# theovincent/iS-DQN

Hardware: AMD Instinct MI355X
Metric: gradient-steps/sec (batch=256, K=9, 84x84x4) (higher is better)
Workload: dtype bf16x3 (split-bf16 MFMA operands hi+lo, fp32 accumulate)

## Files before the change

__graft_entry__.py:

```python
import importlib.util
import os
import sys

ROOT = os.path.dirname(os.path.abspath(__file__))
PKG = os.path.join(ROOT, "is-dqn_amd")
for _p in (ROOT, PKG):
    if _p not in sys.path:
        sys.path.insert(0, _p)


def _build_module():
    spec = importlib.util.spec_from_file_location("isdqn_build", os.path.join(PKG, "build.py"))
    mod = importlib.util.module_from_spec(spec)
    spec.loader.exec_module(mod)
    return mod


def build() -> None:
    from concurrent.futures import ThreadPoolExecutor

    mod = _build_module()
    with ThreadPoolExecutor(4) as pool:
        jobs = [pool.submit(mod.build, verbose=True),
                pool.submit(mod.build, verbose=True, variant="bounds", defines=("ISDQN_BOUNDS",)),
                pool.submit(mod.build, verbose=True, variant="nopair", defines=("ISDQN_NO_U8_PAIR",)),
                pool.submit(mod.build, verbose=True, variant="dev", defines=("ISDQN_DEV",))]
        lib_path = jobs[0].result()
        for j in jobs[1:]:
            j.result()
    from slimdqn import _hip

    handle = _hip.lib()
    for name in _hip.PUBLIC_SYMBOLS:
        getattr(handle, name)
    import slimdqn.networks.isdqn
    import slimdqn.sample_collection.replay_buffer
    import slimdqn.sample_collection.samplers
    import slimdqn.sample_collection.sum_tree

    print(f"built {lib_path}: {handle.isdqn_version().decode()}")


def smoke() -> None:
    import numpy as np
    import torch

    from oracle.isdqn import iSDQN as Oracle
    from oracle.replay_buffer import ReplayBuffer as ORB, TransitionElement as OT
    from oracle.samplers import PrioritizedSamplingDistribution as OP
    from slimdqn.networks.isdqn import iSDQN
    from slimdqn.sample_collection.replay_buffer import ReplayBuffer, TransitionElement
    from slimdqn.sample_collection.samplers import PrioritizedSamplingDistribution

    assert torch.cuda.is_available(), "smoke() needs a GPU"
    K, A, B, feats = 3, 6, 8, [16, 16, 16, 32]
    agent = iSDQN(0, (84, 84, 4), A, K, feats, True, False, "cnn", 1e-3, 0.99, 3, 1, 4, adam_eps=1.5e-4, batch_size=B)
    oracle = Oracle(0, (84, 84, 4), A, K, feats, True, False, "cnn", 1e-3, 0.99, 3, 1, 4, adam_eps=1.5e-4,
                    params=agent.get_model()["params"]["params"])
    rb = ReplayBuffer(PrioritizedSamplingDistribution(1, 64), B, 64, update_horizon=3, gamma=0.99)
# ... 24 lines not shown
```

is-dqn_amd/csrc/gemm_core.h:

```cpp
#pragma once
#include <cstdio>
#include <cstdlib>
#include <type_traits>
#include "common.h"

namespace isdqn {

typedef __attribute__((ext_vector_type(8))) __bf16 bf16x8;
typedef __attribute__((ext_vector_type(4))) short s16x4;
typedef __attribute__((ext_vector_type(8))) short s16x8;
typedef __attribute__((ext_vector_type(4))) float f32x4;

constexpr int GEMM_BK = 32;
constexpr int GEMM_THREADS = 256;

__device__ __forceinline__ int xcd_remap(int bid, int n_blocks) {
    const int xcd = bid & 7, q = n_blocks >> 3, r = n_blocks & 7;
    const int base = xcd < r ? xcd * (q + 1) : r * (q + 1) + (xcd - r) * q;
    return base + (bid >> 3);
}

#define LDS_AS __attribute__((address_space(3)))

__device__ __forceinline__ void split8(const float (&v)[8], bf16x8& hi, bf16x8& lo) {
// ... 106 lines not shown
    if constexpr (!TR) {
        return *reinterpret_cast<const bf16x8*>(tile + (row0 + (lane & 15)) * PITCH + (lane >> 4) * 8);
    } else {
        const int g = lane >> 4, i = lane & 15, q = i >> 2, p = i & 3;
        const __bf16* a0 = tile + (16 * (g >> 1) + 2 * q + (g & 1)) * PITCH + row0 + 4 * p;
        const __bf16* a1 = a0 + 8 * PITCH;
        s16x4 lo = __builtin_amdgcn_ds_read_tr16_b64_v4i16((LDS_AS s16x4*)a0);
        s16x4 hi = __builtin_amdgcn_ds_read_tr16_b64_v4i16((LDS_AS s16x4*)a1);
        s16x8 r = __builtin_shufflevector(lo, hi, 0, 1, 2, 3, 4, 5, 6, 7);
        return __builtin_bit_cast(bf16x8, r);
    }
}

template <class P, class = void>
struct KGroupsOf { static constexpr int value = 1; };
template <class P>
struct KGroupsOf<P, std::void_t<decltype(P::KG)>> { static constexpr int value = P::KG; };
template <class P, class = void>
struct TrPadAOf { static constexpr int value = 16; };
template <class P>
struct TrPadAOf<P, std::void_t<decltype(P::TR_PAD_A)>> { static constexpr int value = P::TR_PAD_A; };
template <class P, class = void>
struct TrPadBOf { static constexpr int value = 16; };
template <class P>
struct TrPadBOf<P, std::void_t<decltype(P::TR_PAD_B)>> { static constexpr int value = P::TR_PAD_B; };
template <class P, class = void>
struct AS8Of { static constexpr bool value = false; };
template <class P>
struct AS8Of<P, std::void_t<decltype(P::A_S8)>> { static constexpr bool value = P::A_S8; };
template <class P, class = void>
struct BS8Of { static constexpr bool value = false; };
template <class P>
struct BS8Of<P, std::void_t<decltype(P::B_S8)>> { static constexpr bool value = P::B_S8; };

template <class P>
struct GemmTraits {
    static constexpr int BM = P::BM, BN = P::BN, WM = P::WM, WN = P::WN;
    static constexpr int MT = BM / WM / 16, NT = BN / WN / 16;
    static constexpr int PASSES = P::PASSES;
    static constexpr int A_PLANES = PASSES >= 2 ? 2 : 1;
    static constexpr int B_PLANES = PASSES >= 3 ? 2 : 1;
    using GA = TileGeom<BM, P::A_TR, TrPadAOf<P>::value>;
    using GB = TileGeom<BN, P::B_TR, TrPadBOf<P>::value>;
    static constexpr int STAGE_ELEMS = A_PLANES * GA::ELEMS + B_PLANES * GB::ELEMS;
    static constexpr int KG = KGroupsOf<P>::value;
    static constexpr int PIPE_BYTES = KG * 2 * STAGE_ELEMS * 2;
    static constexpr int XCHG_BYTES = KG > 1 ? KG * 4 * NT * 4 * 64 * 4 : 0;
    static constexpr int EPI_BYTES = P::EPI_LDS_BYTES + XCHG_BYTES;
    static constexpr int LDS_BYTES = PIPE_BYTES > EPI_BYTES ? PIPE_BYTES : EPI_BYTES;
};

template <class P>
__global__ __launch_bounds__(GEMM_THREADS * KGroupsOf<P>::value) void gemm_kernel(const P p) {
    ISDQN_EMPTY_KERNEL_RETURN
    using T = GemmTraits<P>;
    constexpr int KG = T::KG;
    using GA = typename T::GA;
    using GB = typename T::GB;
    constexpr int MT = T::MT, NT = T::NT, PASSES = T::PASSES;
    extern __shared__ __attribute__((aligned(16))) char smem_raw[];
    __bf16* smem = reinterpret_cast<__bf16*>(smem_raw);

    typename P::Tile tile;
    if (!p.tile((int)blockIdx.x, tile)) return;

    const int kg = KG > 1 ? (int)threadIdx.x / GEMM_THREADS : 0;
    const int tid = (int)threadIdx.x - kg * GEMM_THREADS;
    const int lane = tid & 63;
    const int wave = tid >> 6;
    const int wm = wave / P::WN, wn = wave % P::WN;
    const int wave_m = wm * (MT * 16), wave_n = wn * (NT * 16);

    typename P::ACtx actx[GA::PER_THREAD];
    typename P::BCtx bctx[GB::PER_THREAD];
    int a_lds[GA::PER_THREAD], a_var[GA::PER_THREAD];
    int b_lds[GB::PER_THREAD], b_var[GB::PER_THREAD];
    bool a_on[GA::PER_THREAD], b_on[GB::PER_THREAD];
#pragma unroll
    for (int i = 0; i < GA::PER_THREAD; ++i) {
        int c = tid + i * GEMM_THREADS;
        a_on[i] = c < GA::CHUNKS;
        if (!a_on[i]) c = 0;
        if constexpr (!P::A_TR) {
            int r = stash_row(c), kc = c & 3;
            actx[i] = p.a_ctx(tile, tile.m0 + r);
            a_var[i] = kc * 8;
            a_lds[i] = r * GA::PITCH + kc * 8;
        } else {
            int kk = c / (T::BM / 8), rc = c % (T::BM / 8);
            actx[i] = p.a_ctx(tile, tile.m0 + rc * 8);
            a_var[i] = kk;
            a_lds[i] = tr_row(kk) * GA::PITCH + rc * 8;
        }
    }
#pragma unroll
    for (int i = 0; i < GB::PER_THREAD; ++i) {
// ... 59 lines not shown
#pragma unroll
    for (int mt = 0; mt < MT; ++mt)
#pragma unroll
        for (int nt = 0; nt < NT; ++nt) mfma_init(acc[mt][nt]);

    auto compute = [&](int stage) {
        const __bf16* base = smem + (kg * 2 + stage) * T::STAGE_ELEMS;
        const __bf16* a_hi = base;
        const __bf16* a_lo = base + GA::ELEMS;
        const __bf16* b_hi = base + T::A_PLANES * GA::ELEMS;
        const __bf16* b_lo = b_hi + GB::ELEMS;
        bf16x8 fa_hi[MT], fa_lo[MT];
#pragma unroll
        for (int mt = 0; mt < MT; ++mt) {
            fa_hi[mt] = read_frag<P::A_TR, GA::PITCH>(a_hi, wave_m + mt * 16, lane);
            if constexpr (PASSES >= 2) fa_lo[mt] = read_frag<P::A_TR, GA::PITCH>(a_lo, wave_m + mt * 16, lane);
        }
#pragma unroll
        for (int nt = 0; nt < NT; ++nt) {
            bf16x8 fb_hi = read_frag<P::B_TR, GB::PITCH>(b_hi, wave_n + nt * 16, lane);
            bf16x8 fb_lo;
            if constexpr (PASSES >= 3) fb_lo = read_frag<P::B_TR, GB::PITCH>(b_lo, wave_n + nt * 16, lane);
#pragma unroll
            for (int mt = 0; mt < MT; ++mt) {
                if constexpr (PASSES >= 3)
                    mfma_acc(acc[mt][nt], fa_hi[mt], fb_lo);
                if constexpr (PASSES >= 2)
                    mfma_acc(acc[mt][nt], fa_lo[mt], fb_hi);
                mfma_acc(acc[mt][nt], fa_hi[mt], fb_hi);
            }
        }
    };

    const int nsteps = ((tile.k1 - tile.k0 + GEMM_BK - 1) / GEMM_BK + KG - 1) / KG;
    if (nsteps > 0) {
        fetch(tile.k0 + kg * GEMM_BK);
        stash(0);
        __syncthreads();
        for (int s = 0; s < nsteps; ++s) {
            const bool more = s + 1 < nsteps;
            if (more) fetch(tile.k0 + ((s + 1) * KG + kg) * GEMM_BK);
            compute(s & 1);
            if (more) stash((s + 1) & 1);
            __syncthreads();
        }
    }
    if constexpr (KG > 1) {
        static_assert(KG == 2 && MT == 2, "one row tile per K group");
        float* red = reinterpret_cast<float*>(smem_raw + P::EPI_LDS_BYTES);
#pragma unroll
        for (int nt = 0; nt < NT; ++nt)
#pragma unroll
            for (int r = 0; r < 4; ++r) {
                const float give = kg == 0 ? acc[1][nt][r] : acc[0][nt][r];
                red[(((kg * 4 + wave) * NT + nt) * 4 + r) * 64 + lane] = give;
            }
        __syncthreads();
        f32x4 mine[1][NT];
#pragma unroll
        for (int nt = 0; nt < NT; ++nt)
#pragma unroll
            for (int r = 0; r < 4; ++r) {
                const float got = red[((((1 - kg) * 4 + wave) * NT + nt) * 4 + r) * 64 + lane];
                mine[0][nt][r] = (kg == 0 ? acc[0][nt][r] : acc[1][nt][r]) + got;
            }
        p.epilogue(tile, mine, tile.m0 + wave_m + kg * 16, tile.n0 + wave_n, lane, smem_raw);
    } else {
        p.epilogue(tile, acc, tile.m0 + wave_m, tile.n0 + wave_n, lane, smem_raw);
    }
}

template <class P>
static int launch_gemm(const P& p, int n_blocks, hipStream_t stream) {
    using T = GemmTraits<P>;
    static LdsConfigured configured;
    int rc = ensure_dynamic_lds(&gemm_kernel<P>, T::LDS_BYTES, configured);
    if (rc) return rc;
    ISDQN_REPORT_OCCUPANCY((&gemm_kernel<P>), GEMM_THREADS * T::KG, T::LDS_BYTES, n_blocks);
    if (n_blocks <= 0) return ISDQN_OK;
    hipLaunchKernelGGL(gemm_kernel<P>, dim3(n_blocks), dim3(GEMM_THREADS * T::KG), T::LDS_BYTES, stream, p);
    ISDQN_HIP_CHECK(hipGetLastError());
    return ISDQN_OK;
}

__device__ __forceinline__ void zero8(float (&v)[8]) {
#pragma unroll
    for (int i = 0; i < 8; ++i) v[i] = 0.f;
}
__device__ __forceinline__ float row16_sum(float x) {
    auto dpp = [](float v, auto ctrl) {
        return __builtin_bit_cast(float, __builtin_amdgcn_update_dpp(0, __builtin_bit_cast(int, v), decltype(ctrl)::value, 0xF, 0xF, true));
    };
    x += dpp(x, std::integral_constant<int, 0xB1>{});
    x += dpp(x, std::integral_constant<int, 0x4E>{});
    x += dpp(x, std::integral_constant<int, 0x124>{});
    x += dpp(x, std::integral_constant<int, 0x128>{});
    return x;
}

static __device__ const float isdqn_zero_block[16] = {0.f, 0.f, 0.f, 0.f, 0.f, 0.f, 0.f, 0.f,
                                                      0.f, 0.f, 0.f, 0.f, 0.f, 0.f, 0.f, 0.f};
__device__ __forceinline__ const float* zero_chunk() { return isdqn_zero_block; }

#if defined(ISDQN_BOUNDS)
struct BoundsTable {
    int n, bad, bad_site, pad;
    unsigned long long bad_addr;
    unsigned long long lo[64], hi[64];
};
static __device__ BoundsTable isdqn_bounds;
__device__ __forceinline__ void bounds_check(const void* p, int bytes, int site) {
    const unsigned long long a = (unsigned long long)p, b = a + (unsigned)bytes;
    const unsigned long long z = (unsigned long long)isdqn_zero_block;
// ... 71 lines not shown
```

is-dqn_amd/csrc/learn_step.h:

```cpp
#pragma once
struct SideStream {
    hipStream_t stream = nullptr;
    hipEvent_t ev[2 * MAX_LAYERS + 4];
    int n_ev = 0;
    std::atomic<unsigned> next{0};
    std::atomic<int> state{0};
};
static SideStream* side_stream() {
    static SideStream per_dev[ISDQN_MAX_DEVICES];
    if (ISDQN_DEV_ENV("ISDQN_SINGLE_STREAM")) return nullptr;
    SideStream& s = per_dev[current_device_slot()];
    int st = s.state.load(std::memory_order_acquire);
    if (st == 2) return &s;
    if (st == -1) return nullptr;
    int expected = 0;
    if (s.state.compare_exchange_strong(expected, 1)) {
        bool ok = hipStreamCreateWithFlags(&s.stream, hipStreamNonBlocking) == hipSuccess;
        s.n_ev = 2 * MAX_LAYERS + 4;
        for (int i = 0; ok && i < s.n_ev; ++i) ok = hipEventCreateWithFlags(&s.ev[i], hipEventDisableTiming) == hipSuccess;
        s.state.store(ok ? 2 : -1, std::memory_order_release);
        return ok ? &s : nullptr;
    }
    while ((st = s.state.load(std::memory_order_acquire)) == 1) {}
    return st == 2 ? &s : nullptr;
// ... 139 lines not shown
static int learn_loss(const LearnCtx& c) {
    const bool tnet = (c.double_q || c.munchausen) && c.target_params != nullptr;
    if (!c.hc_S) {
        int rc = loss_and_finalize(c.P, c, c.double_q, tnet ? c.ws + c.P.out_t_off + (c.munchausen ? (int64_t)c.B * c.P.nlog_p : 0) : nullptr,
                                   (tnet && c.munchausen) ? c.ws + c.P.out_t_off : nullptr);
        if (rc || !(c.learn() && c.P.dueling)) return rc;
        const Plan& P = c.P;
        const int w = P.head_nb > 0 ? P.head_nb : 1;
        const int64_t threads = (int64_t)(c.B + 1) * P.n_heads * w;
        hipLaunchKernelGGL(duel_backward_kernel, dim3((unsigned)((threads + DUEL_THREADS - 1) / DUEL_THREADS)), dim3(DUEL_THREADS), 0, c.st,
                           (const float*)(c.ws + P.dout_off), P.nlog_p, c.ws + P.dout_raw_off, P.raw_p, (const float*)(c.ws + P.dbh_off),
                           c.ws + P.dbh_raw_off, c.B, P.n_heads, P.n_actions, w);
        ISDQN_HIP_CHECK(hipGetLastError());
        return ISDQN_OK;
    }
    if (int rc = launch_head_chain(c)) return rc;
    return c.ss ? ISDQN_OK : head_chain_sums(c, c.st);
}

struct WgradJob {
    int layer = -1;
    hipStream_t stream = nullptr;
    hipEvent_t wait = nullptr;
    const float* dz = nullptr;
    int dz_ld = 0;
};

static int dense_wgrad_fused_adam(const LearnCtx& c, const Layer& l, const float* act_in, const WgradJob& j) {
    const MatSrc A{j.dz, j.dz_ld, c.B, l.out_p, 1};
    const MatSrc Bm{act_in, l.in_p, c.B, l.in_p, 1};
    AdamFuse af{c.params + l.w_off, c.adam_m + l.w_off, c.adam_v + l.w_off, c.ws + c.P.adam_tab_off,
                c.cfg->learning_rate, c.cfg->adam_b1, c.cfg->adam_b2, c.cfg->adam_eps,
                c.grad_out ? c.grad_out + l.w_off : nullptr, c.ws + c.P.wsplit_off + l.w_off, c.update() ? 1 : 0, c.wd(1)};
    if (l.is_head)
        return c.x3 ? launch_plain<64, 64, 2, 2, true, true, 3, true, false, true, 2>(A, nullptr, 0, Bm, nullptr, l.in_p, l.out_p, l.in_p, c.B, 1, 0,
                                                                                      j.stream, &af)
                    : launch_plain<64, 64, 2, 2, true, true, 1, true, false, true, 2>(A, nullptr, 0, Bm, nullptr, l.in_p, l.out_p, l.in_p, c.B, 1, 0,
                                                                                      j.stream, &af);
    return c.x3 ? launch_plain<64, 64, 2, 2, true, true, 3, true, false, true, DZ_S8 | 2>(A, nullptr, 0, Bm, nullptr, l.in_p, l.out_p, l.in_p, c.B, 1,
                                                                                          0, j.stream, &af)
                : launch_plain<64, 64, 2, 2, true, true, 1, true, false, true, DZ_S8 | 2>(A, nullptr, 0, Bm, nullptr, l.in_p, l.out_p, l.in_p, c.B, 1,
                                                                                          0, j.stream, &af);
}

static int weight_gradient(const LearnCtx& c, const WgradJob& j, AdamList* adam) {
    const Layer& l = c.P.L[j.layer];
    float* ws = c.ws;
    const float* act_in = j.layer > 0 ? ws + c.P.L[j.layer - 1].act_off : nullptr;
    int w_slabs, rc;
    if (l.is_head && c.hc_S && c.ss) {
        w_slabs = effective_splits(c.B, l.gw_slabs);
    } else if (l.kind == 0) {
        rc = conv_wgrad(l, c.x3, c.in, act_in, j.dz, ws + l.gw_off, c.B, j.stream, &w_slabs);
        if (rc) return rc;
    } else {
        w_slabs = effective_splits(c.B, l.gw_slabs);
        if (w_slabs == 1 && !l.in_unpadded_ld && !c.P.grad_clip) return dense_wgrad_fused_adam(c, l, act_in, j);
        rc = dense_wgrad(l, c.x3, c.in, act_in, j.dz, j.dz_ld, ws + l.gw_off, c.B, j.stream);
        if (rc) return rc;
    }
    adam[c.ss && j.stream == c.wst ? 1 : 0].add(l.w_off, l.w_size, ws + l.gw_off, w_slabs, l.w_size, c.wd(l.kind == 0 ? 0 : 1));
    return ISDQN_OK;
}

#if !defined(ISDQN_FORK_LATE_MAX_B)
#define ISDQN_FORK_LATE_MAX_B 768
#endif
struct BackwardSchedule {
    const LearnCtx& c;
    AdamList* const adam;
    const bool tail_swap, fork_late;
    bool prio_pending, head_pending;
    hipEvent_t head_event = nullptr;
    bool forked = false, layer0_chained = false;
    WgradJob deferred;
// ... 324 lines not shown
```

is-dqn_amd/csrc/net_launch.h:

```cpp
#pragma once
#if defined(ISDQN_DEV)
static long long* g_stamps = nullptr;
static int g_stamp_layer = -1;
static char g_stamp_name[32] = "";
extern "C" int isdqn_debug_set_stamps(void* buf, const char* layer_name) {
    g_stamps = (long long*)buf;
    g_stamp_layer = buf ? 0 : -1;
    snprintf(g_stamp_name, sizeof(g_stamp_name), "%s", layer_name ? layer_name : "");
    return ISDQN_OK;
}
static long long* stamps_for(const char* kernel_tag) {
    return (g_stamp_layer >= 0 && strcmp(kernel_tag, g_stamp_name) == 0) ? g_stamps : nullptr;
}
#else
static long long* stamps_for(const char*) { return nullptr; }
#endif

__global__ __launch_bounds__(256) void split_params_kernel(const float* __restrict__ p, float* __restrict__ mirror, int64_t n_groups) {
    const int64_t g = (int64_t)blockIdx.x * 256 + threadIdx.x;
    if (g >= n_groups) return;
    float v[8];
    load8_aligned(p + g * 8, v);
    s8_store_group(mirror + g * 8, v);
}
// ... 110 lines not shown
    if (passes == 3) return mt == 2 ? launch_conv_fwd_img<2, 3, false>(ip, st)
                          : kg2 ? launch_conv_fwd_img<4, 3, false, 2>(ip, st) : launch_conv_fwd_img<4, 3, false>(ip, st);
    return mt == 2 ? launch_conv_fwd_img<2, 1, false>(ip, st)
         : kg2 ? launch_conv_fwd_img<4, 1, false, 2>(ip, st) : launch_conv_fwd_img<4, 1, false>(ip, st);
}

static int conv_fwd(const Layer& l, bool x3, const float* params, const float* wmir, const NetInput& in, const float* act_in, int n_img,
                    int z_img, float* act, float* z, hipStream_t st) {
    bool done = false;
    int rc = conv_fwd_img(l, x3, params, wmir, in, act_in, n_img, z_img, act, z, st, &done);
    if (rc || done) return rc;
    const bool small = l.cout_p <= 32;
    if (l.is_u8) {
        if (x3) return small ? launch_conv_fwd<32, 2, true>(l, params, wmir, in, act_in, n_img, z_img, act, z, st)
                             : launch_conv_fwd<64, 2, true>(l, params, wmir, in, act_in, n_img, z_img, act, z, st);
        return small ? launch_conv_fwd<32, 1, true>(l, params, wmir, in, act_in, n_img, z_img, act, z, st)
                     : launch_conv_fwd<64, 1, true>(l, params, wmir, in, act_in, n_img, z_img, act, z, st);
    }
    if (x3) return small ? launch_conv_fwd<32, 3, false>(l, params, wmir, in, act_in, n_img, z_img, act, z, st)
                         : launch_conv_fwd<64, 3, false>(l, params, wmir, in, act_in, n_img, z_img, act, z, st);
    return small ? launch_conv_fwd<32, 1, false>(l, params, wmir, in, act_in, n_img, z_img, act, z, st)
                 : launch_conv_fwd<64, 1, false>(l, params, wmir, in, act_in, n_img, z_img, act, z, st);
}

static int effective_splits(int K, int splits, int* steps_per_split = nullptr) {
    int ksteps = ceil_div(K, GEMM_BK);
    if (splits < 1) splits = 1;
    if (splits > ksteps) splits = ksteps;
    int sps = ceil_div(ksteps, splits);
    if (steps_per_split) *steps_per_split = sps;
    return ceil_div(ksteps, sps);
}

template <int BM, int BN, int WM, int WN, bool ATR, bool BTR, int PASSES, bool AL, bool A2PART, bool ADAM = false, int S8M = 0>
static int launch_plain(const MatSrc& A, const float* A2, int a_split, const MatSrc& B, float* C, int ldc, int M,
                        int N, int K, int splits, int64_t slab_stride, hipStream_t st,
                        const AdamFuse* adam = nullptr) {
    PlainGemm<BM, BN, WM, WN, ATR, BTR, PASSES, AL, A2PART, ADAM, S8M> p;
    if (adam) p.adam = *adam;
    p.A = A; p.B = B; p.A2 = A2; p.a_split = a_split; p.C = C; p.ldc = ldc; p.M = M; p.N = N; p.K = K;
    p.tiles_m = ceil_div(M, BM); p.tiles_n = ceil_div(N, BN);
    p.splits = effective_splits(K, splits, &p.steps_per_split);
    p.slab_stride = slab_stride;
    return launch_gemm(p, p.tiles_m * p.tiles_n * p.splits, st);
}

template <bool ATR, bool BTR, bool AL = true, bool A2PART = false, int S8M = 0>
static int plain_big(bool x3, const MatSrc& A, const float* A2, int a_split, const MatSrc& B, float* C, int ldc,
                     int M, int N, int K, int splits, int64_t slab_stride, hipStream_t st) {
    if (x3)
        return launch_plain<128, 128, 2, 2, ATR, BTR, 3, AL, A2PART, false, S8M>(A, A2, a_split, B, C, ldc, M, N, K, splits,
                                                                                 slab_stride, st);
    return launch_plain<128, 128, 2, 2, ATR, BTR, 1, AL, A2PART, false, S8M>(A, A2, a_split, B, C, ldc, M, N, K, splits,
                                                                             slab_stride, st);
}

template <bool ATR, bool BTR, int S8M = 0>
static int plain_narrow(bool x3, const MatSrc& A, const MatSrc& B, float* C, int ldc, int M, int N, int K, int splits,
                        int64_t slab_stride, hipStream_t st) {
    if (x3) return launch_plain<128, 64, 2, 2, ATR, BTR, 3, true, false, false, S8M>(A, nullptr, 0, B, C, ldc, M, N, K, splits, slab_stride, st);
    return launch_plain<128, 64, 2, 2, ATR, BTR, 1, true, false, false, S8M>(A, nullptr, 0, B, C, ldc, M, N, K, splits, slab_stride, st);
}

static int dense_fwd(const Layer& l, bool x3, const float* params, const float* wmir, const NetInput& in, const float* act_in, int rows,
                     int z_rows, float* slab, float* act, float* z, hipStream_t st, bool skip_post = false) {
    MatSrc A, B;
    const float* A2 = nullptr;
    int a_split = 0;
    if (l.in_unpadded_ld) {
        A = MatSrc{in.obs, l.in_unpadded_ld, rows, l.in_f, 0};
        if (in.obs2) { A2 = in.obs2; a_split = in.obs_split; }
    } else {
        A = MatSrc{act_in, l.in_p, rows, l.in_p, 1};
    }
    B = MatSrc{wmir + l.w_off, l.in_p, l.out_f, l.in_p, 1};
    const int ns = effective_splits(l.in_unpadded_ld ? l.in_f : l.K, l.fwd_splits);
    const int64_t slab_stride = l.out_p;
// ... 520 lines not shown
```

is-dqn_amd/csrc/net_problems.h:

```cpp
#pragma once
#include "gemm_core.h"

namespace isdqn {

struct FrameSrc {
    const uint8_t* frames;
    int64_t stride;
    const int* ids;
    int stack;
    int paired_B;
    int H, W;
    int id_pitch = 0, id_off = 0;
    __device__ __forceinline__ int frame_id(int j, int c) const {
#if defined(ISDQN_DEV)
        if (ids == nullptr) return j * stack + c;
#endif
        if (paired_B > 0) {
            const int* q = j < paired_B ? ids + (int64_t)j * 2 * stack + c : ids + (int64_t)(j - paired_B) * 2 * stack + stack + c;
            ISDQN_BOUNDS_CHECK(q, 4, 4);
            return *q;
        }
        ISDQN_BOUNDS_CHECK(ids + (int64_t)j * (id_pitch ? id_pitch : stack) + id_off + c, 4, 4);
        return ids[(int64_t)j * (id_pitch ? id_pitch : stack) + id_off + c];
    }
// ... 20 lines not shown
        patch8_cvt(u, d, v);
    }
    __device__ __forceinline__ void patch8(int j, int c, int iy, int ix0, float (&v)[8]) const {
        patch8_id(frame_id(j, c), iy, ix0, v);
    }
};

struct AdamFuse {
    float *p, *m, *v;
    const float* consts;
    float lr, b1, b2, eps;
    float* grad_out;
    float* mirror;
    int update;
    float wd = 0.f;
};

template <int BM_, int BN_, int WM_, int WN_, bool ATR, bool BTR, int PASSES_, bool AL = true, bool A2PART = false,
          bool ADAM = false, int S8M = 0>
struct PlainGemm {
    static constexpr int BM = BM_, BN = BN_, WM = WM_, WN = WN_, PASSES = PASSES_;
    static constexpr bool A_TR = ATR, B_TR = BTR;
    static constexpr bool A_S8 = (S8M & 1) != 0, B_S8 = (S8M & 2) != 0;
    static constexpr int TR_PAD_B = ADAM ? 8 : 16;
    MatSrc A, B;
    const float* A2;
    int a_split;
    float* C;
    int ldc, M, N, K;
    int tiles_m, tiles_n, splits, steps_per_split;
    int64_t slab_stride;
    AdamFuse adam;
    static constexpr int EPI_LDS_BYTES = ADAM ? BM_ * (BN_ + 4) * 4 : 0;
    struct Tile { int m0, n0, k0, k1, split; };
    struct ACtx { int fixed; };
    struct BCtx { int fixed; };
    __device__ __forceinline__ bool tile(int bid, Tile& t) const {
        bid = xcd_remap(bid, tiles_m * tiles_n * splits);
        int tm = bid % tiles_m, rest = bid / tiles_m;
        int tn = rest % tiles_n;
        t.split = rest / tiles_n;
#if defined(ISDQN_ADAM_ROWMAJOR)
        if constexpr (ADAM) {
            tn = bid % tiles_n;
            tm = bid / tiles_n;
        }
#endif
        if (t.split >= splits) return false;
        t.m0 = tm * BM;
        t.n0 = tn * BN;
        t.k0 = t.split * steps_per_split * GEMM_BK;
        t.k1 = min(K, t.k0 + steps_per_split * GEMM_BK);
        return true;
    }
    __device__ __forceinline__ ACtx a_ctx(const Tile&, int fixed) const { return ACtx{fixed}; }
    __device__ __forceinline__ BCtx b_ctx(const Tile&, int fixed) const { return BCtx{fixed}; }
    __device__ __forceinline__ void load_a(const Tile&, const ACtx& c, int var, float (&v)[8]) const {
        if constexpr (!ATR) {
            if constexpr (A2PART) {
                const bool second = c.fixed >= a_split;
                MatSrc s = A;
                s.base = second ? A2 : A.base;
                s.outer = second ? A.outer - a_split : min(A.outer, a_split);
                s.load<AL || A_S8>(second ? c.fixed - a_split : c.fixed, var, v);
            } else {
                A.load<AL || A_S8>(c.fixed, var, v);
            }
        } else {
            A.load<AL || A_S8>(var, c.fixed, v);
        }
    }
    __device__ __forceinline__ void load_b(const Tile&, const BCtx& c, int var, float (&v)[8]) const {
        if constexpr (!BTR) B.load<AL || B_S8>(c.fixed, var, v);
        else B.load<AL || B_S8>(var, c.fixed, v);
    }
    template <int MT, int NT>
    __device__ __forceinline__ void epilogue(const Tile& t, f32x4 (&acc)[MT][NT], int m_wave, int n_wave, int lane, char* smem) const {
        if constexpr (ADAM) {
            constexpr int LD = BN + 4;
            float* tg = reinterpret_cast<float*>(smem);
            const int lm = m_wave - t.m0, ln = n_wave - t.n0;
            constexpr int N_IT = BM * (BN / 4) / GEMM_THREADS;
            static_assert(BM * (BN / 4) % GEMM_THREADS == 0, "whole float4 rounds");
            const int tid = threadIdx.x;
            f32x4 pm[N_IT], pv[N_IT], pp[N_IT];
            int64_t off[N_IT];
            bool on[N_IT];
#pragma unroll
            for (int it = 0; it < N_IT; ++it) {
                const int i = tid + it * GEMM_THREADS;
                const int rl = i / (BN / 4), c4 = (i % (BN / 4)) * 4;
                const int row = t.m0 + rl, col = t.n0 + c4;
                on[it] = row < M && col < N;
                off[it] = on[it] ? (int64_t)row * ldc + col : 0;
                ISDQN_BOUNDS_CHECK(adam.m + off[it], 16, 10);
                ISDQN_BOUNDS_CHECK(adam.v + off[it], 16, 10);
                ISDQN_BOUNDS_CHECK(adam.p + off[it], 16, 10);
#if !defined(ISDQN_NO_STREAMING)
                pm[it] = __builtin_nontemporal_load((const ISDQN_GLOBAL f32x4*)(adam.m + off[it]));
                pv[it] = __builtin_nontemporal_load((const ISDQN_GLOBAL f32x4*)(adam.v + off[it]));
                pp[it] = __builtin_nontemporal_load((const ISDQN_GLOBAL f32x4*)(adam.p + off[it]));
#else
                pm[it] = *(const ISDQN_GLOBAL f32x4*)(adam.m + off[it]);
                pv[it] = *(const ISDQN_GLOBAL f32x4*)(adam.v + off[it]);
                pp[it] = *(const ISDQN_GLOBAL f32x4*)(adam.p + off[it]);
#endif
            }
#pragma unroll
            for (int mt = 0; mt < MT; ++mt)
#pragma unroll
                for (int nt = 0; nt < NT; ++nt)
#pragma unroll
                    for (int r = 0; r < 4; ++r)
                        tg[(lm + mt * 16 + (lane >> 4) * 4 + r) * LD + ln + nt * 16 + (lane & 15)] = acc[mt][nt][r];
            __syncthreads();
            const float inv_c1 = 1.f / adam.consts[0], inv_c2 = 1.f / adam.consts[1];
#pragma unroll
            for (int it = 0; it < N_IT; ++it) {
                const int i = tid + it * GEMM_THREADS;
                const int rl = i / (BN / 4), c4 = (i % (BN / 4)) * 4;
                const float4 g = *reinterpret_cast<const float4*>(tg + rl * LD + c4);
                const float* gp = &g.x;
                f32x4 nm, nv, np;
#pragma unroll
                for (int r = 0; r < 4; ++r) {
                    float mm = pm[it][r], vv = pv[it][r];
                    np[r] = adam_element(mm, vv, pp[it][r], gp[r], adam.b1, adam.b2, adam.lr, adam.eps, inv_c1, inv_c2);
                    nm[r] = mm;
                    nv[r] = vv;
                }
                if (adam.wd != 0.f) {
#pragma unroll
                    for (int r = 0; r < 4; ++r) np[r] = adamw_decay(np[r], pp[it][r], adam.lr, adam.wd);
                }
                if (on[it] && adam.grad_out) *reinterpret_cast<float4*>(adam.grad_out + off[it]) = g;
                if (on[it] && adam.update) {
#if !defined(ISDQN_NO_STREAMING)
                    __builtin_nontemporal_store(nm, (ISDQN_GLOBAL f32x4*)(adam.m + off[it]));
                    __builtin_nontemporal_store(nv, (ISDQN_GLOBAL f32x4*)(adam.v + off[it]));
                    __builtin_nontemporal_store(np, (ISDQN_GLOBAL f32x4*)(adam.p + off[it]));
#else
                    *reinterpret_cast<f32x4*>(adam.m + off[it]) = nm;
                    *reinterpret_cast<f32x4*>(adam.v + off[it]) = nv;
                    *reinterpret_cast<f32x4*>(adam.p + off[it]) = np;
#endif
                    s8_store_quad(adam.mirror, (int)off[it], np[0], np[1], np[2], np[3]);
                }
            }
            return;
        }
        float* c = C + (int64_t)t.split * slab_stride;
#pragma unroll
        for (int mt = 0; mt < MT; ++mt)
#pragma unroll
            for (int nt = 0; nt < NT; ++nt) {
                int col = n_wave + nt * 16 + (lane & 15);
#pragma unroll
                for (int r = 0; r < 4; ++r) {
                    int row = m_wave + mt * 16 + (lane >> 4) * 4 + r;
                    if (row < M && col < N) c[(int64_t)row * ldc + col] = acc[mt][nt][r];
                }
            }
    }
};

template <int PASSES_, int BM_ = 128, int KG_ = 1>
struct DenseDgradLN {
    static constexpr int BM = BM_, BN = 64, WM = 4, WN = 1, PASSES = PASSES_;
    static constexpr int KG = KG_;
    static constexpr bool A_TR = false, B_TR = true;
    static constexpr bool A_S8 = true;
    static constexpr bool B_S8 = true;
    static constexpr int TR_PITCH = 68;
    static constexpr int SP_BYTES = 4 * KG_ * 3 * 64 * 4;
    static constexpr int EPI_LDS_BYTES = SP_BYTES + 4 * KG_ * 16 * TR_PITCH * 4;
    MatSrc A, B;
    const float* z;
    const float *gamma, *beta;
    float* dz_out;
    float* part;
    int ldc, M, N, K, c_in;
// ... 423 lines not shown
```

Before: 4366.

## Make Adam-fused weight-gradient GEMM persistent and interleave Adam state prefetch with K-loop

The Adam-fused GEMM becomes a persistent kernel. A capped grid, about one workgroup per CU, loops over tiles. The Adam m/v/p state loads are spread across the first K-loop iterations instead of being issued all at once in the epilogue. This aims to hide the optimizer-state memory latency behind MFMA work and to cut launch/tail overhead from many small tiles. In exchange, LDS grows when the epilogue and pipeline buffers are separate, and register pressure rises from holding the prefetched state.

```diff
diff --git a/__graft_entry__.py b/__graft_entry__.py
--- a/__graft_entry__.py
+++ b/__graft_entry__.py
@@ -20,11 +20,12 @@
     from concurrent.futures import ThreadPoolExecutor
 
     mod = _build_module()
-    with ThreadPoolExecutor(4) as pool:
+    with ThreadPoolExecutor(5) as pool:
         jobs = [pool.submit(mod.build, verbose=True),
                 pool.submit(mod.build, verbose=True, variant="bounds", defines=("ISDQN_BOUNDS",)),
                 pool.submit(mod.build, verbose=True, variant="nopair", defines=("ISDQN_NO_U8_PAIR",)),
-                pool.submit(mod.build, verbose=True, variant="dev", defines=("ISDQN_DEV",))]
+                pool.submit(mod.build, verbose=True, variant="dev", defines=("ISDQN_DEV",)),
+                pool.submit(mod.build, verbose=True, variant="adam1t", defines=("ISDQN_ADAM_ONE_TILE",))]
         lib_path = jobs[0].result()
         for j in jobs[1:]:
             j.result()
diff --git a/is-dqn_amd/csrc/gemm_core.h b/is-dqn_amd/csrc/gemm_core.h
--- a/is-dqn_amd/csrc/gemm_core.h
+++ b/is-dqn_amd/csrc/gemm_core.h
@@ -162,6 +162,11 @@
 struct BS8Of { static constexpr bool value = false; };
 template <class P>
 struct BS8Of<P, std::void_t<decltype(P::B_S8)>> { static constexpr bool value = P::B_S8; };
+
+template <class P, class = void>
+struct PersistentOf { static constexpr bool value = false; };
+template <class P>
+struct PersistentOf<P, std::void_t<decltype(P::PERSISTENT)>> { static constexpr bool value = P::PERSISTENT; };
 
 template <class P>
 struct GemmTraits {
@@ -177,8 +182,20 @@
     static constexpr int PIPE_BYTES = KG * 2 * STAGE_ELEMS * 2;
     static constexpr int XCHG_BYTES = KG > 1 ? KG * 4 * NT * 4 * 64 * 4 : 0;
     static constexpr int EPI_BYTES = P::EPI_LDS_BYTES + XCHG_BYTES;
-    static constexpr int LDS_BYTES = PIPE_BYTES > EPI_BYTES ? PIPE_BYTES : EPI_BYTES;
+    static constexpr bool PERSIST = PersistentOf<P>::value;
+    static constexpr int LDS_SHARED_BYTES = PIPE_BYTES > EPI_BYTES ? PIPE_BYTES : EPI_BYTES;
+    static constexpr int LDS_BYTES = PERSIST ? PIPE_BYTES + EPI_BYTES : LDS_SHARED_BYTES;
 };
+
+#if defined(ISDQN_DEV)
+#define ISDQN_GEMM_STAMP(cond, slot)                                                                             \
+    if ((cond) && p.stamps != nullptr && threadIdx.x == 0) {                                                     \
+        p.stamps[(int64_t)blockIdx.x * 8 + (slot)] = (long long)__builtin_amdgcn_s_memtime();                    \
+        if ((slot) == 0) p.stamps[(int64_t)blockIdx.x * 8 + 7] = (long long)__builtin_amdgcn_s_memrealtime();    \
+    }
+#else
+#define ISDQN_GEMM_STAMP(cond, slot)
+#endif
 
 template <class P>
 __global__ __launch_bounds__(GEMM_THREADS * KGroupsOf<P>::value) void gemm_kernel(const P p) {
@@ -192,6 +209,9 @@
     __bf16* smem = reinterpret_cast<__bf16*>(smem_raw);
 
     typename P::Tile tile;
+    if constexpr (T::PERSIST) {
+        if ((int)blockIdx.x >= p.n_tiles()) return;
+    }
     if (!p.tile((int)blockIdx.x, tile)) return;
 
     const int kg = KG > 1 ? (int)threadIdx.x / GEMM_THREADS : 0;
@@ -317,6 +337,61 @@
         }
     };
 
+    if constexpr (T::PERSIST) {
+        static_assert(KG == 1, "persistent problems have one K group");
+        char* epi = smem_raw + p.epi_offset;
+        typename P::Prefetch pre;
+        const typename P::Uniform uni = p.uniforms();
+        auto reassign = [&]() {
+#pragma unroll
+            for (int i = 0; i < GA::PER_THREAD; ++i) {
+                const int c = a_on[i] ? tid + i * GEMM_THREADS : 0;
+                actx[i] = p.a_ctx(tile, tile.m0 + (P::A_TR ? (c % (T::BM / 8)) * 8 : stash_row(c)));
+            }
+#pragma unroll
+            for (int i = 0; i < GB::PER_THREAD; ++i) {
+                const int c = b_on[i] ? tid + i * GEMM_THREADS : 0;
+                bctx[i] = p.b_ctx(tile, tile.n0 + (P::B_TR ? (c % (T::BN / 8)) * 8 : stash_row(c)));
+            }
+        };
+        for (int bid = (int)blockIdx.x, round = 0;; ++round) {
+            const int nsteps = (tile.k1 - tile.k0 + GEMM_BK - 1) / GEMM_BK;
+            fetch(tile.k0);
+            stash(0);
+            __syncthreads();
+            ISDQN_GEMM_STAMP(round < 2, round * 3);
+#pragma unroll
+            for (int s = 0; s < P::PRE_ROUNDS; ++s) {
+                const bool live = s < nsteps, more = s + 1 < nsteps;
+                if (more) fetch(tile.k0 + (s + 1) * GEMM_BK);
+                p.prefetch_round(tile, s, pre);
+                if (live) compute(s & 1);
+                if (more) stash((s + 1) & 1);
+                if (live) __syncthreads();
+            }
+            for (int s = P::PRE_ROUNDS; s < nsteps; ++s) {
+                const bool more = s + 1 < nsteps;
+                if (more) fetch(tile.k0 + (s + 1) * GEMM_BK);
+                compute(s & 1);
+                if (more) stash((s + 1) & 1);
+                __syncthreads();
+            }
+            ISDQN_GEMM_STAMP(round < 2, round * 3 + 1);
+            p.stage(tile, acc, tile.m0 + wave_m, tile.n0 + wave_n, lane, epi);
+            __syncthreads();
+            ISDQN_GEMM_STAMP(round == 0, 6);
+            p.apply(tile, pre, uni, epi);
+            ISDQN_GEMM_STAMP(round < 2, round * 3 + 2);
+            bid += p.grid;
+            if (bid >= p.n_tiles() || !p.tile(bid, tile)) break;
+            reassign();
+#pragma unroll
+            for (int mt = 0; mt < MT; ++mt)
+#pragma unroll
+                for (int nt = 0; nt < NT; ++nt) mfma_init(acc[mt][nt]);
+        }
+        return;
+    }
     const int nsteps = ((tile.k1 - tile.k0 + GEMM_BK - 1) / GEMM_BK + KG - 1) / KG;
     if (nsteps > 0) {
         fetch(tile.k0 + kg * GEMM_BK);
@@ -356,14 +431,14 @@
 }
 
 template <class P>
-static int launch_gemm(const P& p, int n_blocks, hipStream_t stream) {
+static int launch_gemm(const P& p, int n_blocks, hipStream_t stream, int lds_bytes = GemmTraits<P>::LDS_BYTES) {
     using T = GemmTraits<P>;
     static LdsConfigured configured;
-    int rc = ensure_dynamic_lds(&gemm_kernel<P>, T::LDS_BYTES, configured);
+    int rc = ensure_dynamic_lds(&gemm_kernel<P>, lds_bytes, configured);
     if (rc) return rc;
-    ISDQN_REPORT_OCCUPANCY((&gemm_kernel<P>), GEMM_THREADS * T::KG, T::LDS_BYTES, n_blocks);
+    ISDQN_REPORT_OCCUPANCY((&gemm_kernel<P>), GEMM_THREADS * T::KG, lds_bytes, n_blocks);
     if (n_blocks <= 0) return ISDQN_OK;
-    hipLaunchKernelGGL(gemm_kernel<P>, dim3(n_blocks), dim3(GEMM_THREADS * T::KG), T::LDS_BYTES, stream, p);
+    hipLaunchKernelGGL(gemm_kernel<P>, dim3(n_blocks), dim3(GEMM_THREADS * T::KG), lds_bytes, stream, p);
     ISDQN_HIP_CHECK(hipGetLastError());
     return ISDQN_OK;
 }
diff --git a/is-dqn_amd/csrc/learn_step.h b/is-dqn_amd/csrc/learn_step.h
--- a/is-dqn_amd/csrc/learn_step.h
+++ b/is-dqn_amd/csrc/learn_step.h
@@ -195,15 +195,18 @@
     AdamFuse af{c.params + l.w_off, c.adam_m + l.w_off, c.adam_v + l.w_off, c.ws + c.P.adam_tab_off,
                 c.cfg->learning_rate, c.cfg->adam_b1, c.cfg->adam_b2, c.cfg->adam_eps,
                 c.grad_out ? c.grad_out + l.w_off : nullptr, c.ws + c.P.wsplit_off + l.w_off, c.update() ? 1 : 0, c.wd(1)};
+    char tag[40];
+    snprintf(tag, sizeof(tag), "adam:%s", l.name);
+    long long* const stamps = stamps_for(tag);
     if (l.is_head)
         return c.x3 ? launch_plain<64, 64, 2, 2, true, true, 3, true, false, true, 2>(A, nullptr, 0, Bm, nullptr, l.in_p, l.out_p, l.in_p, c.B, 1, 0,
-                                                                                      j.stream, &af)
+                                                                                      j.stream, &af, stamps)
                     : launch_plain<64, 64, 2, 2, true, true, 1, true, false, true, 2>(A, nullptr, 0, Bm, nullptr, l.in_p, l.out_p, l.in_p, c.B, 1, 0,
-                                                                                      j.stream, &af);
+                                                                                      j.stream, &af, stamps);
     return c.x3 ? launch_plain<64, 64, 2, 2, true, true, 3, true, false, true, DZ_S8 | 2>(A, nullptr, 0, Bm, nullptr, l.in_p, l.out_p, l.in_p, c.B, 1,
-                                                                                          0, j.stream, &af)
+                                                                                          0, j.stream, &af, stamps)
                 : launch_plain<64, 64, 2, 2, true, true, 1, true, false, true, DZ_S8 | 2>(A, nullptr, 0, Bm, nullptr, l.in_p, l.out_p, l.in_p, c.B, 1,
-                                                                                          0, j.stream, &af);
+                                                                                          0, j.stream, &af, stamps);
 }
 
 static int weight_gradient(const LearnCtx& c, const WgradJob& j, AdamList* adam) {
diff --git a/is-dqn_amd/csrc/net_launch.h b/is-dqn_amd/csrc/net_launch.h
--- a/is-dqn_amd/csrc/net_launch.h
+++ b/is-dqn_amd/csrc/net_launch.h
@@ -166,17 +166,60 @@
     return ceil_div(ksteps, sps);
 }
 
+#if !defined(ISDQN_ADAM_WG_PER_CU)
+#define ISDQN_ADAM_WG_PER_CU 1
+#endif
+#if !defined(ISDQN_ADAM_PERSIST_MAX_K)
+#define ISDQN_ADAM_PERSIST_MAX_K 256
+#endif
+static int adam_grid(int n_tiles, int K) {
+    static int cus[ISDQN_MAX_DEVICES] = {0};
+    const int d = current_device_slot();
+    if (cus[d] == 0) {
+        int dev = 0, n = 0;
+        if (hipGetDevice(&dev) != hipSuccess || hipDeviceGetAttribute(&n, hipDeviceAttributeMultiprocessorCount, dev) != hipSuccess || n < 1) n = 1;
+        cus[d] = n;
+    }
+    int max_k = ISDQN_ADAM_PERSIST_MAX_K;
+#if defined(ISDQN_DEV)
+    if (const char* e = getenv("ISDQN_ADAM_PERSIST_MAX_K")) max_k = atoi(e);
+#endif
+    int grid = n_tiles;
+    const int cap = round_up(ISDQN_ADAM_WG_PER_CU * cus[d], 8);
+    if (K <= max_k && n_tiles > cap) {
+        grid = round_up(ceil_div(n_tiles, ceil_div(n_tiles, cap)), 8);
+        if (grid > cap) grid = cap;
+    }
+#if defined(ISDQN_DEV)
+    if (const char* e = getenv("ISDQN_ADAM_GRID")) grid = atoi(e) > 1 ? atoi(e) : 1;
+#endif
+    return grid;
+}
+
 template <int BM, int BN, int WM, int WN, bool ATR, bool BTR, int PASSES, bool AL, bool A2PART, bool ADAM = false, int S8M = 0>
 static int launch_plain(const MatSrc& A, const float* A2, int a_split, const MatSrc& B, float* C, int ldc, int M,
                         int N, int K, int splits, int64_t slab_stride, hipStream_t st,
-                        const AdamFuse* adam = nullptr) {
-    PlainGemm<BM, BN, WM, WN, ATR, BTR, PASSES, AL, A2PART, ADAM, S8M> p;
+                        const AdamFuse* adam = nullptr, long long* stamps = nullptr) {
+    using Problem = PlainGemm<BM, BN, WM, WN, ATR, BTR, PASSES, AL, A2PART, ADAM, S8M>;
+    Problem p;
     if (adam) p.adam = *adam;
     p.A = A; p.B = B; p.A2 = A2; p.a_split = a_split; p.C = C; p.ldc = ldc; p.M = M; p.N = N; p.K = K;
     p.tiles_m = ceil_div(M, BM); p.tiles_n = ceil_div(N, BN);
     p.splits = effective_splits(K, splits, &p.steps_per_split);
     p.slab_stride = slab_stride;
-    return launch_gemm(p, p.tiles_m * p.tiles_n * p.splits, st);
+    const int n_tiles = p.tiles_m * p.tiles_n * p.splits;
+    if constexpr (Problem::PERSISTENT) {
+        using T = GemmTraits<Problem>;
+        p.grid = adam_grid(n_tiles, K);
+        const bool one_each = p.grid >= n_tiles;
+        p.epi_offset = one_each ? 0 : T::PIPE_BYTES;
+#if defined(ISDQN_DEV)
+        p.stamps = stamps;
+#endif
+        return launch_gemm(p, p.grid, st, one_each ? T::LDS_SHARED_BYTES : T::LDS_BYTES);
+    }
+    (void)stamps;
+    return launch_gemm(p, n_tiles, st);
 }
 
 template <bool ATR, bool BTR, bool AL = true, bool A2PART = false, int S8M = 0>
diff --git a/is-dqn_amd/csrc/net_problems.h b/is-dqn_amd/csrc/net_problems.h
--- a/is-dqn_amd/csrc/net_problems.h
+++ b/is-dqn_amd/csrc/net_problems.h
@@ -76,6 +76,20 @@
     int64_t slab_stride;
     AdamFuse adam;
     static constexpr int EPI_LDS_BYTES = ADAM ? BM_ * (BN_ + 4) * 4 : 0;
+#if defined(ISDQN_ADAM_ONE_TILE)
+    static constexpr bool PERSISTENT = false;
+#else
+    static constexpr bool PERSISTENT = ADAM;
+#endif
+    static constexpr int PRE_ROUNDS = BM_ * (BN_ / 4) / GEMM_THREADS;
+    static_assert(!ADAM || BM_ * (BN_ / 4) % GEMM_THREADS == 0, "whole float4 rounds");
+    struct Prefetch { f32x4 pm[PRE_ROUNDS], pv[PRE_ROUNDS], pp[PRE_ROUNDS]; };
+    int epi_offset = 0;
+    int grid = 0;
+#if defined(ISDQN_DEV)
+    long long* stamps = nullptr;
+#endif
+    __device__ __forceinline__ int n_tiles() const { return tiles_m * tiles_n * splits; }
     struct Tile { int m0, n0, k0, k1, split; };
     struct ACtx { int fixed; };
     struct BCtx { int fixed; };
@@ -118,79 +132,95 @@
         if constexpr (!BTR) B.load<AL || B_S8>(c.fixed, var, v);
         else B.load<AL || B_S8>(var, c.fixed, v);
     }
+    __device__ __forceinline__ void adam_slot(const Tile& t, int it, bool& on, int64_t& off) const {
+        const int i = (int)threadIdx.x + it * GEMM_THREADS;
+        const int rl = i / (BN / 4), c4 = (i % (BN / 4)) * 4;
+        const int row = t.m0 + rl, col = t.n0 + c4;
+        on = row < M && col < N;
+        off = on ? (int64_t)row * ldc + col : 0;
+    }
+    __device__ __forceinline__ void prefetch_round(const Tile& t, int it, Prefetch& pre) const {
+        bool on;
+        int64_t off;
+        adam_slot(t, it, on, off);
+        ISDQN_BOUNDS_CHECK(adam.m + off, 16, 10);
+        ISDQN_BOUNDS_CHECK(adam.v + off, 16, 10);
+        ISDQN_BOUNDS_CHECK(adam.p + off, 16, 10);
+#if !defined(ISDQN_NO_STREAMING)
+        pre.pm[it] = __builtin_nontemporal_load((const ISDQN_GLOBAL f32x4*)(adam.m + off));
+        pre.pv[it] = __builtin_nontemporal_load((const ISDQN_GLOBAL f32x4*)(adam.v + off));
+        pre.pp[it] = __builtin_nontemporal_load((const ISDQN_GLOBAL f32x4*)(adam.p + off));
+#else
+        pre.pm[it] = *(const ISDQN_GLOBAL f32x4*)(adam.m + off);
+        pre.pv[it] = *(const ISDQN_GLOBAL f32x4*)(adam.v + off);
+        pre.pp[it] = *(const ISDQN_GLOBAL f32x4*)(adam.p + off);
+#endif
+    }
+    template <int MT, int NT>
+    __device__ __forceinline__ void stage(const Tile& t, f32x4 (&acc)[MT][NT], int m_wave, int n_wave, int lane, char* smem) const {
+        constexpr int LD = BN + 4;
+        float* tg = reinterpret_cast<float*>(smem);
+        const int lm = m_wave - t.m0, ln = n_wave - t.n0;
+#pragma unroll
+        for (int mt = 0; mt < MT; ++mt)
+#pragma unroll
+            for (int nt = 0; nt < NT; ++nt)
+#pragma unroll
+                for (int r = 0; r < 4; ++r)
+                    tg[(lm + mt * 16 + (lane >> 4) * 4 + r) * LD + ln + nt * 16 + (lane & 15)] = acc[mt][nt][r];
+    }
+    struct Uniform { float inv_c1, inv_c2; };
+    __device__ __forceinline__ Uniform uniforms() const { return Uniform{1.f / adam.consts[0], 1.f / adam.consts[1]}; }
+    __device__ __forceinline__ void apply(const Tile& t, const Prefetch& pre, const Uniform& u, const char* smem) const {
+        constexpr int LD = BN + 4;
+        const float* tg = reinterpret_cast<const float*>(smem);
+        const int tid = threadIdx.x;
+        const float inv_c1 = u.inv_c1, inv_c2 = u.inv_c2;
+#pragma unroll
+        for (int it = 0; it < PRE_ROUNDS; ++it) {
+            const int i = tid + it * GEMM_THREADS;
+            const int rl = i / (BN / 4), c4 = (i % (BN / 4)) * 4;
+            bool on;
+            int64_t off;
+            adam_slot(t, it, on, off);
+            const float4 g = *reinterpret_cast<const float4*>(tg + rl * LD + c4);
+            const float* gp = &g.x;
+            f32x4 nm, nv, np;
+#pragma unroll
+            for (int r = 0; r < 4; ++r) {
+                float mm = pre.pm[it][r], vv = pre.pv[it][r];
+                np[r] = adam_element(mm, vv, pre.pp[it][r], gp[r], adam.b1, adam.b2, adam.lr, adam.eps, inv_c1, inv_c2);
+                nm[r] = mm;
+                nv[r] = vv;
+            }
+            if (adam.wd != 0.f) {
+#pragma unroll
+                for (int r = 0; r < 4; ++r) np[r] = adamw_decay(np[r], pre.pp[it][r], adam.lr, adam.wd);
+            }
+            if (on && adam.grad_out) *reinterpret_cast<float4*>(adam.grad_out + off) = g;
+            if (on && adam.update) {
+#if !defined(ISDQN_NO_STREAMING)
+                __builtin_nontemporal_store(nm, (ISDQN_GLOBAL f32x4*)(adam.m + off));
+                __builtin_nontemporal_store(nv, (ISDQN_GLOBAL f32x4*)(adam.v + off));
+                __builtin_nontemporal_store(np, (ISDQN_GLOBAL f32x4*)(adam.p + off));
+#else
+                *reinterpret_cast<f32x4*>(adam.m + off) = nm;
+                *reinterpret_cast<f32x4*>(adam.v + off) = nv;
+                *reinterpret_cast<f32x4*>(adam.p + off) = np;
+#endif
+                s8_store_quad(adam.mirror, (int)off, np[0], np[1], np[2], np[3]);
+            }
+        }
+    }
     template <int MT, int NT>
     __device__ __forceinline__ void epilogue(const Tile& t, f32x4 (&acc)[MT][NT], int m_wave, int n_wave, int lane, char* smem) const {
         if constexpr (ADAM) {
-            constexpr int LD = BN + 4;
-            float* tg = reinterpret_cast<float*>(smem);
-            const int lm = m_wave - t.m0, ln = n_wave - t.n0;
-            constexpr int N_IT = BM * (BN / 4) / GEMM_THREADS;
-            static_assert(BM * (BN / 4) % GEMM_THREADS == 0, "whole float4 rounds");
-            const int tid = threadIdx.x;
-            f32x4 pm[N_IT], pv[N_IT], pp[N_IT];
-            int64_t off[N_IT];
-            bool on[N_IT];
-#pragma unroll
-            for (int it = 0; it < N_IT; ++it) {
-                const int i = tid + it * GEMM_THREADS;
-                const int rl = i / (BN / 4), c4 = (i % (BN / 4)) * 4;
-                const int row = t.m0 + rl, col = t.n0 + c4;
-                on[it] = row < M && col < N;
-                off[it] = on[it] ? (int64_t)row * ldc + col : 0;
-                ISDQN_BOUNDS_CHECK(adam.m + off[it], 16, 10);
-                ISDQN_BOUNDS_CHECK(adam.v + off[it], 16, 10);
-                ISDQN_BOUNDS_CHECK(adam.p + off[it], 16, 10);
-#if !defined(ISDQN_NO_STREAMING)
-                pm[it] = __builtin_nontemporal_load((const ISDQN_GLOBAL f32x4*)(adam.m + off[it]));
-                pv[it] = __builtin_nontemporal_load((const ISDQN_GLOBAL f32x4*)(adam.v + off[it]));
-                pp[it] = __builtin_nontemporal_load((const ISDQN_GLOBAL f32x4*)(adam.p + off[it]));
-#else
-                pm[it] = *(const ISDQN_GLOBAL f32x4*)(adam.m + off[it]);
-                pv[it] = *(const ISDQN_GLOBAL f32x4*)(adam.v + off[it]);
-                pp[it] = *(const ISDQN_GLOBAL f32x4*)(adam.p + off[it]);
-#endif
-            }
-#pragma unroll
-            for (int mt = 0; mt < MT; ++mt)
-#pragma unroll
-                for (int nt = 0; nt < NT; ++nt)
-#pragma unroll
-                    for (int r = 0; r < 4; ++r)
-                        tg[(lm + mt * 16 + (lane >> 4) * 4 + r) * LD + ln + nt * 16 + (lane & 15)] = acc[mt][nt][r];
+            Prefetch pre;
+#pragma unroll
+            for (int it = 0; it < PRE_ROUNDS; ++it) prefetch_round(t, it, pre);
+            stage(t, acc, m_wave, n_wave, lane, smem);
             __syncthreads();
-            const float inv_c1 = 1.f / adam.consts[0], inv_c2 = 1.f / adam.consts[1];
-#pragma unroll
-            for (int it = 0; it < N_IT; ++it) {
-                const int i = tid + it * GEMM_THREADS;
-                const int rl = i / (BN / 4), c4 = (i % (BN / 4)) * 4;
-                const float4 g = *reinterpret_cast<const float4*>(tg + rl * LD + c4);
-                const float* gp = &g.x;
-                f32x4 nm, nv, np;
-#pragma unroll
-                for (int r = 0; r < 4; ++r) {
-                    float mm = pm[it][r], vv = pv[it][r];
-                    np[r] = adam_element(mm, vv, pp[it][r], gp[r], adam.b1, adam.b2, adam.lr, adam.eps, inv_c1, inv_c2);
-                    nm[r] = mm;
-                    nv[r] = vv;
-                }
-                if (adam.wd != 0.f) {
-#pragma unroll
-                    for (int r = 0; r < 4; ++r) np[r] = adamw_decay(np[r], pp[it][r], adam.lr, adam.wd);
-                }
-                if (on[it] && adam.grad_out) *reinterpret_cast<float4*>(adam.grad_out + off[it]) = g;
-                if (on[it] && adam.update) {
-#if !defined(ISDQN_NO_STREAMING)
-                    __builtin_nontemporal_store(nm, (ISDQN_GLOBAL f32x4*)(adam.m + off[it]));
-                    __builtin_nontemporal_store(nv, (ISDQN_GLOBAL f32x4*)(adam.v + off[it]));
-                    __builtin_nontemporal_store(np, (ISDQN_GLOBAL f32x4*)(adam.p + off[it]));
-#else
-                    *reinterpret_cast<f32x4*>(adam.m + off[it]) = nm;
-                    *reinterpret_cast<f32x4*>(adam.v + off[it]) = nv;
-                    *reinterpret_cast<f32x4*>(adam.p + off[it]) = np;
-#endif
-                    s8_store_quad(adam.mirror, (int)off[it], np[0], np[1], np[2], np[3]);
-                }
-            }
+            apply(t, pre, uniforms(), smem);
             return;
         }
         float* c = C + (int64_t)t.split * slab_stride;
```

Result: no change. 4389 (median of 6 runs) (+0.5%).
